# mmdagent/distantspeechrecognition-mirror

Measured on AMD Instinct MI355X. Metric: decoded_audio_hours_per_sec, higher is better.
Workload: dtype f32

## Files before the change

distantspeechrecognition-mirror_amd/csrc/decoder.cpp:

```cpp
#include "common.h"
#include "wfst_graph.h"
#include "lattice.h"
#include "lexicon.h"
#include "wordtrace.h"
#include "viterbi.h"
#include "decode_plan.h"
#include <algorithm>
#include <cmath>

namespace dsr {

static_assert(kPlanSideBytes == (size_t) kSideLds * sizeof(Side), "decode_plan.h budgets the side records of viterbi.h");

struct DecoderState {
  dsr_decoder_cfg cfg; bool haveGraph = false; int nSlots = 0; int nNodes = 0;
  WfstGraph::Csr csr; WfstGraph::Tables tab;
  DevBuf<int> d_xoff, d_xarc, d_xpathOff, d_eoff, d_path, d_nodeFinal, d_queue; DevBuf<float> d_pathCost;
  DevBuf<XRec> d_xrec; DevBuf<ERec> d_erec; DevBuf<float> d_arcCost, d_nodeCost; DevBuf<uint32_t> d_arcOut, d_arcIn;
  DevBuf<TokA> d_tokA, d_ctok; DevBuf<TokB> d_tokB; DevBuf<Side> d_side; DevBuf<XRecD> d_xrecD; int fastOK = 0; int maxCnt = 0; DevBuf<int> d_tokOff, d_tokCnt, d_owner, d_rank, d_chead; DevBuf<unsigned> d_tags; DevBuf<CandA> d_cA; DevBuf<CandB> d_cB; DevBuf<unsigned> d_first; DevBuf<Bp> d_arena;
  DevBuf<long long> d_prof; DevBuf<dsr_decode_result> d_res; DevBuf<int> d_arcs; DevBuf<unsigned> d_words;
  long arenaCap = 0; int initial = 0; unsigned tokenMemoryLimit = 0;
  long lastPoolCap = 0;
  DevBuf<SegState> d_segState; DevBuf<int> d_segDone; DevBuf<unsigned long long> d_poolNext; DevBuf<TokA> d_saveA; DevBuf<TokB> d_saveB;
  DevBuf<WTok> w_tok; DevBuf<WCand> w_cand; DevBuf<int> w_tokOff, w_rank; DevBuf<unsigned long long> w_best; DevBuf<unsigned> w_first; DevBuf<int4> w_traces; size_t w_tablesFor = 0;
  bool costNegZero = false; double costMinAbs = HUGE_VAL;
  DevBuf<uint4> d_lat; DevBuf<double> d_latTtl; DevBuf<long> d_latFrameOff; DevBuf<int> d_arenaLat; DevBuf<int4> d_latFinal; DevBuf<int> d_latInfo;
  int latU = 0, latTmax = 0; long latArenaCap = 0; WfstGraph graphCopy; DevBuf<TokA> d_tokA3; DevBuf<TokB> d_tokB3;
  const dsr_lexicon* lexIn = nullptr; const dsr_lexicon* lexOut = nullptr; uint32_t eosX = 0; std::string eosSymbol;
  int lastU = 0; size_t lastMaxPath = 0; bool lastPaths = false;
  PinBuf<dsr_decode_result> h_res; PinBuf<int> h_arcs; PinBuf<unsigned> h_words; hipEvent_t evDone = nullptr;
  int pendingU = 0; size_t pendingPath = 0; int pendingSlots = 0; long long* pendingProf = nullptr;
  int dumpOn = 0; long dumpCap = 0; DevBuf<long> d_dumpFrameOff, d_dumpCount; DevBuf<int> d_dumpNode, d_dumpArc; DevBuf<float> d_dumpAc, d_dumpLm;
  std::vector<int64_t> h_dumpFrameOff; std::vector<int32_t> h_dumpNode, h_dumpArc; std::vector<float> h_dumpAc, h_dumpLm; int64_t h_dumpFrames = 0;
};

}

using namespace dsr;
struct dsr_decoder : DecoderState {};

extern "C" {

void dsr_decoder_default_cfg(dsr_decoder_cfg* c)
{ memset(c, 0, sizeof(*c)); c->beam = 100.0; c->lmScale = 12.0; c->lmPenalty = 0.0; c->silPenalty = 0.0; c->silenceX = 0xFFFFFFFFu;
  c->propagateN = 5; c->wordTraceLattice = 1; }

dsr_status dsr_decoder_create(const dsr_decoder_cfg* cfg, dsr_decoder** out)
{
  return guard([&] {
    if (!cfg || !out) throw Error(DSR_E_PARAMETER, "null argument");
    require_device();
    dsr_decoder* d = new dsr_decoder(); d->cfg = *cfg;
    if (d->cfg.maxActive <= 0) d->cfg.maxActive = 65536;
    if (d->cfg.maxCandidates <= 0) d->cfg.maxCandidates = 8 * d->cfg.maxActive;
    if (d->cfg.maxCandidates >= (1 << 24)) throw Error(DSR_E_PARAMETER, "maxCandidates must be < 2^24");
    if (d->cfg.streams <= 0) {
      hipDeviceProp_t prop; int dev = 0; DSR_HIP(hipGetDevice(&dev)); DSR_HIP(hipGetDeviceProperties(&prop, dev));
      d->cfg.streams = prop.multiProcessorCount;
      const int t = read_vit_env().slots; if (t > 0) d->cfg.streams = t;
    }
    *out = d;
  });
}
void dsr_decoder_destroy(dsr_decoder* d) { if (d && d->evDone) (void) hipEventDestroy(d->evDone); delete d; }

dsr_status dsr_decoder_set(dsr_decoder* d, const dsr_wfst* g)
{
  return guard([&] {
    if (!d || !g) throw Error(DSR_E_PARAMETER, "null argument");
    if (g->initial < 0) throw Error(DSR_E_CONSISTENCY, "the transducer has no arcs");
    d->csr = g->csr(); d->tab = g->tables(d->csr, (size_t) 1 << 28);
    d->nNodes = (int) g->nodes.size(); d->initial = g->initial; d->graphCopy = *g;
    std::vector<int> nf(d->nNodes); std::vector<float> nc(d->nNodes);
    for (int i = 0; i < d->nNodes; i++) { nf[i] = g->nodes[i].final_; nc[i] = g->nodes[i].cost; }
    d->d_xoff.upload(d->tab.xoff); d->d_eoff.upload(d->tab.eoff); d->d_path.upload(d->tab.path);
    if (d->tab.xrec.empty()) throw Error(DSR_E_CONSISTENCY, "the transducer has no emitting arcs");
    d->d_xrec.upload(d->tab.xrec); d->d_xarc.upload(d->tab.xarc); d->d_xpathOff.upload(d->tab.xpathOff);
    {
      const size_t nx = d->tab.xrec.size(); std::vector<XRecD> xd(nx); int maxCnt = 0; std::vector<float> pc(1, 0.0f);
      for (size_t r = 0; r < nx; r++) {
        const XRec& x = d->tab.xrec[r]; XRecD& o = xd[r];
        o.dst = x.dst; o.dist = x.dist; o.cost = x.cost; o.meta = x.meta; o.dstXoff = d->tab.xoff[x.dst]; o.dstCnt = d->tab.xoff[x.dst + 1] - d->tab.xoff[x.dst];
        const int po = d->tab.xpathOff[r], plen = (int) (x.meta & 0xFFFFu); o.p2 = 0; o.eps1 = 0.0f;
        if (x.meta >> 18) throw Error(DSR_E_CONSISTENCY, "expansion record %zu: meta bits above 17 are in use", r);
        if (plen) { const int a0 = d->tab.path[po]; o.eps1 = d->csr.cost[a0]; if (d->csr.out[a0] != 0) o.meta |= 0x20000u; }
        if (plen > 14) o.meta |= 0x80000000u;
        else if (plen > 1) {
// ... 167 lines not shown
    DSR_HIP(hipMemsetAsync(d->w_best.p, 0xFF, sizeof(unsigned long long) * S * d->nNodes, st)); DSR_HIP(hipMemsetAsync(d->w_first.p, 0xFF, sizeof(unsigned) * S * d->nNodes, st));
  }
  if (maxPath < 1) maxPath = 1;
  d->d_arcs.reserve((size_t) U * maxPath); d->d_words.reserve((size_t) U * maxPath);
  DSR_HIP(hipMemsetAsync(d->d_queue.p, 0, 8 * sizeof(int), st));
  WtArgs A; A.nNodes = d->nNodes; A.initial = d->initial; A.xoff = d->d_xoff.p; A.xrec = d->d_xrec.p; A.xarc = d->d_xarc.p; A.xpathOff = d->d_xpathOff.p; A.eoff = d->d_eoff.p;
  A.erec = d->d_erec.p; A.path = d->d_path.p; A.arcCost = d->d_arcCost.p; A.arcOut = d->d_arcOut.p; A.arcIn = d->d_arcIn.p; A.nodeFinal = d->d_nodeFinal.p; A.nodeCost = d->d_nodeCost.p;
  A.beam = c.beam; A.lmScale = c.lmScale; A.lmPenalty = c.lmPenalty; A.silPenalty = c.silPenalty; A.silenceX = c.silenceX; A.insertSilence = c.insertSilence;
  A.maxTok = c.maxActive; A.maxCand = c.maxCandidates; A.maxTraces = maxTraces;
  A.tok = d->w_tok.p; A.cand = d->w_cand.p; A.tokOff = d->w_tokOff.p; A.rank = d->w_rank.p; A.bestKey = d->w_best.p; A.firstSlot = d->w_first.p; A.traces = d->w_traces.p; A.queue = d->d_queue.p;
  A.scores = score; A.nframes = nframes; A.U = U; A.Tmax = Tmax; A.nDist = nDist; A.res = d->d_res.p; A.arcsOut = d->d_arcs.p; A.wordsOut = d->d_words.p; A.maxPath = maxPath;
  wordtrace_launch(A, slots, st);
  enqueue_result_copies(d, U, want_paths ? (size_t) U * maxPath : 0, st);
  d->pendingSlots = slots; d->pendingProf = nullptr; d->latU = 0;
}

static VitArgs fill_vit_args(dsr_decoder* d, const DecodePlan& P, const VitEnv& env, const float* score, const int32_t* nframes, int U, int Tmax, int nDist,
                             int maxPath, bool wantPaths, hipStream_t st)
{
  const int slots = P.slots; const bool latOn = d->cfg.latticeTokens > 0;
  d->d_res.reserve(U);
  if (wantPaths) { d->d_arcs.reserve((size_t) U * (maxPath > 0 ? maxPath : 1)); d->d_words.reserve((size_t) U * (maxPath > 0 ? maxPath : 1)); }
  DSR_HIP(hipMemsetAsync(d->d_queue.p, 0, 8 * sizeof(int), st));
  if (d->dumpOn) {
    d->dumpCap = (long) d->cfg.maxActive * 64 < (long) 1 << 26 ? (long) 1 << 24 : (long) 1 << 26;
    d->d_dumpFrameOff.reserve(Tmax + 2); d->d_dumpCount.reserve(2);
    d->d_dumpNode.reserve(d->dumpCap); d->d_dumpArc.reserve(d->dumpCap); d->d_dumpAc.reserve(d->dumpCap); d->d_dumpLm.reserve(d->dumpCap);
    DSR_HIP(hipMemsetAsync(d->d_dumpCount.p, 0, 2 * sizeof(long), st));
  }
  VitArgs A; GraphDev& G = A.G; DecDev& D = A.D;
  G.nNodes = d->nNodes; G.initial = d->initial; G.xoff = d->d_xoff.p; G.xrec = d->d_xrec.p; G.xrecD = d->d_xrecD.p; G.xarc = d->d_xarc.p;
  G.xpathOff = d->d_xpathOff.p; G.eoff = d->d_eoff.p; G.erec = d->d_erec.p; G.path = d->d_path.p; G.pathCost = d->d_pathCost.p; G.arcCost = d->d_arcCost.p;
  G.arcOut = d->d_arcOut.p; G.arcIn = d->d_arcIn.p; G.nodeFinal = d->d_nodeFinal.p; G.nodeCost = d->d_nodeCost.p;
  D.beam = d->cfg.beam; D.lmScale = d->cfg.lmScale; D.lmPenalty = d->cfg.lmPenalty; D.silPenalty = d->cfg.silPenalty;
  D.noPen = (d->cfg.lmScale > 0.0 && std::isfinite(d->cfg.lmScale) && d->cfg.lmScale * d->cfg.lmPenalty == 0.0 && d->cfg.lmScale * d->cfg.silPenalty == 0.0 &&
             !d->costNegZero && (d->costMinAbs == HUGE_VAL || d->cfg.lmScale * d->costMinAbs >= 0x1p-60) && !env.pen) ? 1 : 0;
  D.silenceX = d->cfg.silenceX; D.maxTok = d->cfg.maxActive; D.maxCand = d->cfg.maxCandidates; D.arenaCap = d->arenaCap;
  D.tokA = d->d_tokA.p; D.tokB = d->d_tokB.p; D.ctok = d->d_ctok.p; D.side = d->d_side.p; D.fastOK = d->fastOK; D.tokOff = d->d_tokOff.p; D.owner = d->d_owner.p; D.rank = d->d_rank.p; D.cA = d->d_cA.p; D.cB = d->d_cB.p;
  D.first = d->d_first.p; D.tags = d->d_tags.p; D.tokCnt = d->d_tokCnt.p; D.chead = d->d_chead.p; D.arena = d->d_arena.p; D.queue = d->d_queue.p;
  D.segDrop = env.segDrop; D.segQueues = P.segQueues; D.segFrames = P.segFrames; D.segCount = P.segCount;
  D.poolCap = 0; D.poolChunk = 0; D.poolNext = nullptr; D.segState = nullptr; D.segDone = nullptr; D.saveA = nullptr; D.saveB = nullptr;
  if (P.segFrames > 0) {
    d->d_segState.reserve(U); d->d_segDone.reserve(U); d->d_poolNext.reserve(1);
    d->d_saveA.reserve((size_t) U * d->cfg.maxActive); d->d_saveB.reserve((size_t) U * d->cfg.maxActive);
    DSR_HIP(hipMemsetAsync(d->d_segDone.p, 0, sizeof(int) * (size_t) U, st)); DSR_HIP(hipMemsetAsync(d->d_poolNext.p, 0, sizeof(unsigned long long), st));
    D.poolCap = (long) ((size_t) std::max(P.poolArenas, slots) * (size_t) d->arenaCap); if (D.poolCap > (long) 0xFFFFFFF0L) D.poolCap = (long) 0xFFFFFFF0L;
    D.poolChunk = std::min<long>(262144, std::max<long>(4096, D.poolCap / (4 * (long) U)));
    D.poolNext = d->d_poolNext.p; D.segState = d->d_segState.p; D.segDone = d->d_segDone.p; D.saveA = d->d_saveA.p; D.saveB = d->d_saveB.p;
  }
  d->lastPoolCap = D.poolCap;
  D.prof = nullptr;
  if (env.prof) { d->d_prof.reserve((size_t) slots * kProfN); D.prof = d->d_prof.p; }
  D.dumpOn = d->dumpOn; D.dumpCap = d->dumpCap; D.dumpFrameOff = d->d_dumpFrameOff.p; D.dumpNode = d->d_dumpNode.p; D.dumpAc = d->d_dumpAc.p;
  D.dumpLm = d->d_dumpLm.p; D.dumpArc = d->d_dumpArc.p; D.dumpCount = d->d_dumpCount.p;
  D.topN = d->cfg.topN > 0 ? d->cfg.topN : 0; D.tokA3 = nullptr; D.tokB3 = nullptr;
  if (D.topN > 0) { d->d_tokA3.reserve((size_t) slots * d->cfg.maxActive); d->d_tokB3.reserve((size_t) slots * d->cfg.maxActive); D.tokA3 = d->d_tokA3.p; D.tokB3 = d->d_tokB3.p; }
  D.latOn = latOn ? 1 : 0; D.latCap = 0; D.lat = nullptr; D.latTtl = nullptr; D.latFrameOff = nullptr; D.arenaLat = nullptr; D.latFinal = nullptr; D.latInfo = nullptr;
  if (latOn) {
    const size_t cap = (size_t) d->cfg.latticeTokens;
    d->d_lat.reserve((size_t) U * cap); d->d_latTtl.reserve((size_t) U * cap); d->d_latFrameOff.reserve((size_t) U * (Tmax + 3));
    d->d_arenaLat.reserve((size_t) U * (size_t) d->arenaCap); d->d_latFinal.reserve((size_t) U * d->cfg.maxActive); d->d_latInfo.reserve((size_t) 4 * U);
    DSR_HIP(hipMemsetAsync(d->d_latInfo.p, 0, sizeof(int) * 4 * (size_t) U, st));
    D.latCap = (long) cap; D.lat = d->d_lat.p; D.latTtl = d->d_latTtl.p; D.latFrameOff = d->d_latFrameOff.p; D.arenaLat = d->d_arenaLat.p; D.latFinal = d->d_latFinal.p; D.latInfo = d->d_latInfo.p;
    d->latU = U; d->latTmax = Tmax; d->latArenaCap = d->arenaCap;
  } else d->latU = 0;
  A.scores = score; A.nframesArr = nframes; A.U = U; A.Tmax = Tmax; A.nDist = nDist; A.res = d->d_res.p;
  A.arcsOut = wantPaths ? d->d_arcs.p : nullptr; A.wordsOut = wantPaths ? d->d_words.p : nullptr; A.maxPath = maxPath;
  A.useLdsRow = P.useLdsRow; A.hashN = P.hashN; A.regionB = (int) (kSideLds * sizeof(Side)); A.cntCap = P.cntCap;
  return A;
}

dsr_status dsr_decoder_decode_launch(dsr_decoder* d, const float* score, const int32_t* nframes, int U, int Tmax, int nDist,
                                     int maxPath, int want_paths, void* stream)
{
  return guard([&] {
    if (!d || !score || !nframes) throw Error(DSR_E_PARAMETER, "null argument");
    if (!d->haveGraph) throw Error(DSR_E_INITIALIZATION, "call set() with a transducer first");
    if (d->pendingU > 0) throw Error(DSR_E_CONSISTENCY, "a decode is already in flight on this decoder: collect it first");
    if (U <= 0) return;
    hipStream_t st = (hipStream_t) stream;
    if (d->cfg.wordTrace) { launch_wordtrace(d, score, nframes, U, Tmax, nDist, maxPath, want_paths, st); return; }
    check_arc_inputs(d, nDist);
    const bool latOn = d->cfg.latticeTokens > 0;
    if (latOn && d->dumpOn) throw Error(DSR_E_PARAMETER, "lattice bookkeeping and the token dump are separate debugging aids: enable one");
    const VitEnv env = read_vit_env();
    PlanIn in; in.streams = d->cfg.streams; in.maxActive = d->cfg.maxActive; in.arenaTokens = d->cfg.arenaTokens; in.latticeTokens = d->cfg.latticeTokens;
    in.topN = d->cfg.topN; in.dumpOn = d->dumpOn != 0; in.nNodes = d->nNodes; in.maxCnt = d->maxCnt; in.U = U; in.Tmax = Tmax; in.nDist = nDist;
    in.staticLds = viterbi_static_lds(plan_base_modes(in, env));
    const DecodePlan P = plan_decode(in, env, [&] { return xcd_round_robin(st); });
    ensure_scratch(d, P.slots, Tmax, latOn ? U : (P.segFrames > 0 ? P.poolArenas : 0));
    if (maxPath < 0) maxPath = 0;
    const VitArgs A = fill_vit_args(d, P, env, score, nframes, U, Tmax, nDist, maxPath, want_paths != 0, st);
    if (env.segVerbose) fprintf(stderr, "[dsr viterbi] %d utterances on %d workgroups: %s, %s state table\n", U, P.slots, P.segFrames > 0 ? (P.segQueues == 8 ? "time-sliced, XCD-bound queues" : "time-sliced, one queue") : "run to completion", P.narrow ? "narrow" : "wide");
    viterbi_launch(P.modes, A, P.slots, P.ldsBytes, st);
    enqueue_result_copies(d, U, want_paths ? (size_t) U * maxPath : 0, st);
    d->pendingSlots = P.slots; d->pendingProf = A.D.prof;
  });
}

static void report_profile(const long long* prof, int slots)
{
  std::vector<long long> hp((size_t) slots * kProfN); DSR_HIP(hipMemcpy(hp.data(), prof, hp.size() * sizeof(long long), hipMemcpyDeviceToHost));
  double acc[32] = {0}; for (int s2 = 0; s2 < slots; s2++) for (int i = 0; i < 32; i++) acc[i] += (double) hp[(size_t) s2 * kProfN + i];
  fprintf(stderr, "[dsr viterbi prof] mean us per slot:");
  for (int i = 0; i < 32; i++) if (i != 15) fprintf(stderr, " p%d=%.0f", i, acc[i] / slots / 100.0);
  fprintf(stderr, "\n");
  double tmin = 1e30, tmax = 0.0, tsum = 0.0;
  for (int s2 = 0; s2 < slots; s2++) { double t = 0.0; for (int i = 0; i < 32; i++) if (i != 15) t += (double) hp[(size_t) s2 * kProfN + i]; t /= 100.0; tsum += t; if (t < tmin) tmin = t; if (t > tmax) tmax = t; }
  {
    double h[12] = {0}; for (int s2 = 0; s2 < slots; s2++) for (int i = 0; i < 12; i++) h[i] += (double) hp[(size_t) s2 * kProfN + 32 + i];
    const double nf = h[0] + h[1] + h[2] + h[3], tk = h[4] + h[5] + h[6] + h[7];
    static const char* const cn[4] = {"<=8192", "<=12288", ">12288", "memory path"};
    for (int c = 0; c < 4; c++) if (h[c] > 0) fprintf(stderr, "[dsr viterbi prof] frames with %s placements: %.1f %% of the frames, %.1f %% of the frame time, %.1f us per frame, %.2f ns per placement\n",
                                                      cn[c], 100.0 * h[c] / nf, 100.0 * h[4 + c] / tk, h[4 + c] / 100.0 / h[c], h[4 + c] * 10.0 / h[8 + c]);
  }
  fprintf(stderr, "[dsr viterbi prof] busy us per slot: mean %.0f min %.0f max %.0f\n", tsum / slots, tmin, tmax);
  if (slots >= 64 && slots % 8 == 0) {
// ... 163 lines not shown
```

distantspeechrecognition-mirror_amd/csrc/k_viterbi.hip:

```cpp
#include "viterbi.h"
#include <algorithm>
#include <cmath>
#include <type_traits>

namespace dsr {

static constexpr uint32_t kNone = 0xFFFFFFFFu;
static constexpr uint32_t kEndBit = 0x80000000u;
static constexpr int kWaves = kThreads / 64;
static constexpr int kFastK = 8;
static constexpr int kB = 2;
static constexpr int kFastE = 8190;
static constexpr int kP1 = 16;
static constexpr int kW = 4;

typedef const __attribute__((address_space(4))) VitArgs* KP;

__device__ __forceinline__ unsigned ld_u32(const unsigned* p) { return __hip_atomic_load(p, __ATOMIC_RELAXED, __HIP_MEMORY_SCOPE_AGENT); }
__device__ __forceinline__ int ld_i32(const int* p) { return __hip_atomic_load(p, __ATOMIC_RELAXED, __HIP_MEMORY_SCOPE_AGENT); }
__device__ __forceinline__ void st_u32(unsigned* p, unsigned v) { __hip_atomic_store(p, v, __ATOMIC_RELAXED, __HIP_MEMORY_SCOPE_AGENT); }
__device__ __forceinline__ void st_i32(int* p, int v) { __hip_atomic_store(p, v, __ATOMIC_RELAXED, __HIP_MEMORY_SCOPE_AGENT); }
__device__ __forceinline__ void st_u64_dev(void* p, unsigned long long v) { __hip_atomic_store(reinterpret_cast<unsigned long long*>(p), v, __ATOMIC_RELAXED, __HIP_MEMORY_SCOPE_AGENT); }
__device__ __forceinline__ unsigned long long ld_u64_dev(const void* p) { return __hip_atomic_load(reinterpret_cast<const unsigned long long*>(p), __ATOMIC_RELAXED, __HIP_MEMORY_SCOPE_AGENT); }

// ... 92 lines not shown
__global__ __launch_bounds__(kThreads) void k_viterbi(const VitArgs argsInKernarg)
{
  (void) argsInKernarg;
  constexpr bool PROF = (MODES & 1) != 0, EXTRA = (MODES & 2) != 0;
  constexpr bool NARROW = (MODES & 4) != 0;
  const KP KA = (KP) __builtin_amdgcn_kernarg_segment_ptr();
  KP ka = KA;
#define RELOAD() do { ka = KA; asm volatile("" : "+s"(ka)); } while (0)
  RELOAD();
  extern __shared__ __attribute__((aligned(16))) unsigned char smem[];
  float* srow = reinterpret_cast<float*>(smem);
  const int useLdsRow = ka->useLdsRow, nDist = ka->nDist, hashN = ka->hashN, regionB = ka->regionB, cntCap = ka->cntCap;
  unsigned* hkey = reinterpret_cast<unsigned*>(srow + (useLdsRow ? ((nDist + 3) & ~3) : 4));
  unsigned* hfirst = hkey + hashN;
  unsigned* const tab = hkey; const int tabN = NARROW ? 2 * hashN : hashN;
  Side* sideL = reinterpret_cast<Side*>(hfirst + hashN);
  unsigned short* cntL = reinterpret_cast<unsigned short*>(reinterpret_cast<unsigned char*>(hfirst + hashN) + regionB);
  __shared__ int s_waveTot[kWaves];
  __shared__ int s_waveTotE[kWaves];
  __shared__ double s_waveMin[kWaves];
  __shared__ float s_waveMag[kWaves];
  __shared__ unsigned long long s_waveKey[kWaves];
  __shared__ int s_sideN;
  __shared__ int s_tb[2];
  __shared__ unsigned s_bm[kFastC / 32];
  __shared__ unsigned s_gbase[kFastC / 64 + 4];
  __shared__ int s_cnt[(kFastK + 32) * kWaves];
  __shared__ int s_err;
  __shared__ long long s_prof[32]; __shared__ long long s_tlast;
  __shared__ long long s_hist[PROF ? 12 : 1]; __shared__ long long s_tfr;
  __shared__ long long s_stat[3];
  __shared__ int s_maxActive; __shared__ unsigned s_tag; __shared__ long long s_latOff;
  if (PROF && threadIdx.x < 32) s_prof[threadIdx.x] = 0;
  if (PROF && threadIdx.x < 12) s_hist[threadIdx.x] = 0;
#define TICK(ix) do { if (PROF && tid == 0) { const long long tn = (long long) wall_clock64(); s_prof[ix] += tn - s_tlast; s_tlast = tn; } } while (0)
  constexpr int nthr = kThreads, nw = kWaves;
  __shared__ int s_u, s_seg, s_help; __shared__ long long s_chunk;

  const int tid = threadIdx.x;
  const int slot = blockIdx.x;
#define TOKA(ix) ((EXTRA && (ix) == 2) ? ka->D.tokA3 + (size_t) slot * ka->D.maxTok : ka->D.tokA + ((size_t) slot * 2 + (size_t) (ix)) * ka->D.maxTok)
#define TOKB(ix) ((EXTRA && (ix) == 2) ? ka->D.tokB3 + (size_t) slot * ka->D.maxTok : ka->D.tokB + ((size_t) slot * 2 + (size_t) (ix)) * ka->D.maxTok)
#define curA TOKA(bufCur)
#define nxtA TOKA(bufNxt)
#define curB TOKB(bufCur)
#define nxtB TOKB(bufNxt)
#define sprA TOKA(bufSpr)
#define sprB TOKB(bufSpr)
#define ctok (ka->D.ctok + (size_t) slot * 8192)
#define side (ka->D.side + (size_t) slot * kFastC)
#define cA (ka->D.cA + (size_t) slot * ka->D.maxCand)
#define cB (ka->D.cB + (size_t) slot * ka->D.maxCand)
  if (tid == 0) s_tag = ka->D.tags[slot];
#define arena (ka->D.arena + (size_t) ((EXTRA && ka->D.latOn) ? u : (ka->D.segFrames > 0 ? 0 : slot)) * ka->D.arenaCap)
#define sc (ka->scores + (size_t) u * ka->Tmax * nDist)
  constexpr int fastCapC = ((kFastK + 32) * nthr < kFastC) ? (kFastK + 32) * nthr : kFastC;
  constexpr int fastCapN = kP1 * 64 * nw;
  const bool fastOK = ka->D.fastOK && hashN >= 8192;
  const int tableC = (tabN >> 1) + (tabN >> 2), regC = NARROW ? tableC : 2 * tableC, eCap = kFastE, sideLds = regionB >> 5;

  const int nq = (EXTRA || ka->D.segFrames <= 0) ? 1 : ka->D.segQueues;
  const int xcd = nq == 8 ? (int) (__builtin_amdgcn_s_getreg((3 << 11) | 20) & 7u) : 0;
  if (tid == 0) s_help = (nq == 8 && ((ka->D.segDrop >> xcd) & 1)) ? 1 : 0;
  for (;;) {
    __syncthreads();
    if (tid == 0) {
      const int segS0 = EXTRA ? 0 : ka->D.segFrames; int help = s_help, uu = -1, sg = 0;
      for (;;) {
        const int qx = (xcd + help) & (nq - 1), Uq = (ka->U - qx + nq - 1) / nq;
        int it = -1;
        if (help == 0) { it = atomicAdd(ka->D.queue + qx, 1); if (it >= (segS0 > 0 ? ka->D.segCount * Uq : Uq)) it = -1; }
        else {
          int c = ld_i32(ka->D.queue + qx);
          while (c < Uq) { const int prev = atomicCAS(ka->D.queue + qx, c, c + 1); if (prev == c) { it = c; break; } c = prev; }
        }
        if (it >= 0) { uu = segS0 > 0 ? qx + nq * (it % Uq) : it; sg = segS0 > 0 ? it / Uq : 0; break; }
        if (segS0 > 0 && nq == 8 && help < 7) help++; else break;
      }
      if (uu >= 0 && help > 0) { st_i32(&ka->D.segState[uu].status, -2); asm volatile("s_waitcnt vmcnt(0)" ::: "memory"); st_i32(&ka->D.segDone[uu], 0x7FFFFFFF); sg = -1; }
      s_help = help; s_u = uu; s_seg = sg;
    }
    __syncthreads();
    RELOAD();
    const int segS = EXTRA ? 0 : ka->D.segFrames;
    const int u = s_u; if (u < 0) break;
    const bool whole = s_seg < 0; const int seg = whole ? 0 : s_seg;
    const int T = ka->nframesArr[u] < ka->Tmax ? ka->nframesArr[u] : ka->Tmax;
    const int fr0 = seg * segS, frEnd = (segS > 0 && !whole) ? fr0 + segS : 0x7FFFFFFF;
    if (fr0 > T) continue;
    if (EXTRA && ka->D.latOn && tid == 0) ka->D.latFrameOff[(size_t) u * (ka->Tmax + 3)] = 0;
    if (PROF && tid == 0) { const long long tn = (long long) wall_clock64(); if (s_prof[15]) s_prof[10] += tn - s_prof[15]; s_tlast = tn; }
#define dump (EXTRA && ka->D.dumpOn && slot == 0)

    int status = DSR_OK;
// ... 10 lines not shown
        TokB b0; b0.node = ka->G.initial; b0.cnt = ka->G.xoff[ka->G.initial + 1] - ka->G.xoff[ka->G.initial]; curB[0] = b0;
      }
    } else {
      if (tid == 0) { while (ld_i32(&ka->D.segDone[u]) < seg) __builtin_amdgcn_s_sleep(16); }
      __syncthreads();
      if (nq == 1) __builtin_amdgcn_fence(__ATOMIC_ACQUIRE, "agent");
      const SegState* const sst = ka->D.segState + u;
      status = ld_i32(&sst->status);
      if (status != DSR_OK) continue;
      n = ld_i32(&sst->n); arenaOff = (long) ld_u64_dev(&sst->arenaOff); chunkEnd = (long) ld_u64_dev(&sst->chunkEnd); arenaUsed = (long) ld_u64_dev(&sst->arenaUsed); thresh = __longlong_as_double((long long) ld_u64_dev(&sst->thresh));
      if (tid == 0) { s_stat[0] = (long long) ld_u64_dev(&sst->stat[0]); s_stat[1] = (long long) ld_u64_dev(&sst->stat[1]); s_stat[2] = (long long) ld_u64_dev(&sst->stat[2]); s_maxActive = ld_i32(&sst->maxActive); s_latOff = 0; }
      const TokA* const svA = ka->D.saveA + (size_t) u * ka->D.maxTok; const TokB* const svB = ka->D.saveB + (size_t) u * ka->D.maxTok;
      for (int i = tid; i < n; i += nthr) {
        const unsigned long long a0 = ld_u64_dev(&svA[i]), a1 = ld_u64_dev(reinterpret_cast<const unsigned long long*>(&svA[i]) + 1), b0 = ld_u64_dev(&svB[i]);
        unsigned long long* da = reinterpret_cast<unsigned long long*>(&curA[i]); da[0] = a0; da[1] = a1; *reinterpret_cast<unsigned long long*>(&curB[i]) = b0;
      }
    }
    __syncthreads();

    bool cntOK = false;
    int preC = -1;
    const bool preRow = useLdsRow && nDist <= 2 * nthr;
    float rowNext[2] = {0.0f, 0.0f};
    if (preRow && fr0 < T) { const float* r0 = sc + (size_t) fr0 * nDist; if (tid < nDist) rowNext[0] = r0[tid]; if (tid + nthr < nDist) rowNext[1] = r0[tid + nthr]; }
    TICK(11);
    int fr = fr0;
    for (; fr <= T && fr < frEnd && status == DSR_OK; fr++) {
      RELOAD();
      int tidO = (int) threadIdx.x; asm volatile("" : "+v"(tidO));
      const int tid = tidO, lane = tid & 63, wave = tid >> 6;
      const int mode = (fr == T) ? 1 : 0;
      if (mode == 0 && useLdsRow) {
        if (preRow) {
          if (tid < nDist) srow[tid] = rowNext[0];
          if (tid + nthr < nDist) srow[tid + nthr] = rowNext[1];
          if (fr + 1 < T) {
            const float* nr = sc + (size_t) (fr + 1) * nDist;
            if (tid < nDist) rowNext[0] = nr[tid];
            if (tid + nthr < nDist) rowNext[1] = nr[tid + nthr];
          }
        } else { for (int i = tid; i < nDist; i += nthr) srow[i] = sc[(size_t) fr * nDist + i]; }
      }
      const float* rowG = sc + (size_t) fr * nDist;
      int numNew = 0, numStat = -1;
      if (fr > 0) TICK(23);
      if (PROF && tid == 0) { s_tlast = (long long) wall_clock64(); s_tfr = s_tlast; }
      bool fast = fastOK && mode == 0 && n <= fastCapN && !(EXTRA && (ka->D.latOn || ka->D.topN > 0));
// ... 836 lines not shown
          if (tid == 0) { ka->D.dumpFrameOff[fr] = o; ka->D.dumpFrameOff[fr + 1] = o + numNew; cnt[0] = o + numNew; cnt[1] = fr + 1; }
        }
        if (numStat < 0) numStat = numNew;
        if (numStat == 0 || numNew == 0) { status = DSR_E_CONSISTENCY; break; }
        { const int t = bufCur; bufCur = bufNxt; bufNxt = t; }
        n = numNew; arenaOff += numNew; arenaUsed += numNew;
        if (tid == nthr - 1) { s_stat[0] += numStat; s_stat[1] += Cfr; if (fast) s_stat[2] += 1; if (numStat > s_maxActive) s_maxActive = numStat; }
        thresh = __dadd_rn(topScore, ka->D.beam);
      } else {
        const TokA* lst = numNew > 0 ? nxtA : curA; const int cntL = numNew > 0 ? numNew : n;
        unsigned long long key = ~0ull;
        for (int i = tid; i < cntL; i += nthr) {
          const TokA t = lst[i]; const float s = __fadd_rn(t.ac, t.lm);
          if (s == s) { const unsigned long long k = ((unsigned long long) f2ord(s) << 32) | (unsigned) i; if (k < key) key = k; }
        }
        key = wave_min_u64(key);
        if (lane == 0) s_waveKey[wave] = key;
        if (EXTRA && ka->D.latOn) {
          const TokB* lstB = numNew > 0 ? nxtB : curB; int4* lf = ka->D.latFinal + (size_t) u * ka->D.maxTok;
          for (int i = tid; i < cntL; i += nthr) { const TokA t = ld_tok(&lst[i]); lf[i] = make_int4(lstB[i].node, (int) t.bp, __float_as_int(t.ac), __float_as_int(t.lm)); }
          if (tid == 0) { int* li = ka->D.latInfo + 4 * (size_t) u; li[0] = cntL; li[1] = numNew > 0 ? 1 : 0; li[2] = (int) (arenaOff + (numNew > 0 ? numNew : 0)); li[3] = T; }
        }
        __syncthreads();
        int* hopRec = reinterpret_cast<int*>(cB); const int hopCap = 2 * ka->D.maxCand; int* hopOff = hopRec + hopCap;
        if (tid == 0) {
          dsr_decode_result* const res = ka->res;
          clear_result(&res[u]); dsr_decode_result& r = res[u];
          unsigned long long k = ~0ull; for (int w = 0; w < nw; w++) if (s_waveKey[w] < k) k = s_waveKey[w];
          r.frames = T - 1; r.reachedFinal = numNew > 0 ? 1 : 0; r.finalStatesN = numNew;  r.activeHypos = (long) s_stat[0]; r.placements = (long) s_stat[1] + Cfr; r.registerFrames = (long) s_stat[2]; r.maxActiveSeen = s_maxActive; r.status = DSR_OK;
          int nH = 0;
          if (k != ~0ull) {
            const TokA bt = ld_tok(&lst[(unsigned) (k & 0xFFFFFFFFu)]);
            r.ac = bt.ac; r.lm = bt.lm; r.score = __dadd_rn((double) bt.ac, (double) bt.lm);
            for (uint32_t bq = bt.bp; bq != kNone && nH < hopCap; ) {
              uint2 e; if (segS > 0) { const unsigned long long v = ld_u64_dev(&arena[bq]); e.x = (unsigned) v; e.y = (unsigned) (v >> 32); } else e = *reinterpret_cast<const uint2*>(&arena[bq]);
              hopRec[nH++] = (int) e.y; bq = e.x;
            }
          } else r.status = DSR_E_CONSISTENCY;
          s_tb[0] = nH; s_tb[1] = 0;
        }
        __syncthreads();
        const int nH = s_tb[0];
        auto block_excl = [&](const int v, int& total) -> int {
          const int incl = wave_incl_scan(v, lane);
          if (lane == 63) s_waveTot[wave] = incl;
          __syncthreads();
          int base = 0, tot = 0;
          for (int w = 0; w < nw; w++) { const int q = s_waveTot[w]; if (w < wave) base += q; tot += q; }
          __syncthreads();
          total = tot; return base + incl - v;
        };
        int nA = 0;
        for (int b0 = 0; b0 < nH; b0 += nthr) {
          const int i = b0 + tid; int len = 0;
          if (i < nH) { const uint32_t rc = (uint32_t) hopRec[i]; len = (rc & kEndBit) ? ka->G.erec[rc & ~kEndBit].pathLen : (int) (ka->G.xrec[rc].meta & 0xFFFFu) + 1; }
          int total; const int ex = block_excl(len, total);
          if (i < nH) hopOff[i] = nA + ex;
          nA += total;
        }
        int* const arcsOut = ka->arcsOut; unsigned* const wordsOut = ka->wordsOut; const int maxPath = ka->maxPath; dsr_decode_result* const res = ka->res;
        int* ao = arcsOut ? arcsOut + (size_t) u * maxPath : nullptr;
        int nWloc = 0;
        for (int i = tid; i < nH; i += nthr) {
          const uint32_t rc = (uint32_t) hopRec[i]; int pos = nA - hopOff[i];
          if (rc & kEndBit) {
            const ERec e = ka->G.erec[rc & ~kEndBit];
            for (int h = e.pathLen - 1; h >= 0; h--) { const int a = ka->G.path[e.pathOff + h]; pos--; if (ao && pos < maxPath) ao[pos] = a; if (ka->G.arcOut[a] != 0) nWloc++; }
          } else {
            const int a = ka->G.xarc[rc]; pos--; if (ao && pos < maxPath) ao[pos] = a; if (ka->G.arcOut[a] != 0) nWloc++;
            const int pl = (int) (ka->G.xrec[rc].meta & 0xFFFFu); const int po = ka->G.xpathOff[rc];
            for (int h = pl - 1; h >= 0; h--) { const int a2 = ka->G.path[po + h]; pos--; if (ao && pos < maxPath) ao[pos] = a2; if (ka->G.arcOut[a2] != 0) nWloc++; }
          }
        }
        if (nWloc) atomicAdd(&s_tb[1], nWloc);
        __syncthreads();
        if (wordsOut && ao) {
          unsigned* wo = wordsOut + (size_t) u * maxPath; int q = 0;
          const int lim = nA < maxPath ? nA : maxPath;
          for (int b0 = 0; b0 < lim; b0 += nthr) {
            const int i = b0 + tid; unsigned o = 0u;
            if (i < lim) o = ka->G.arcOut[ao[i]];
            int total; const int ex = block_excl(o != 0u ? 1 : 0, total);
            if (o != 0u && q + ex < maxPath) wo[q + ex] = o;
            q += total;
          }
        }
        if (tid == 0) {
          if (res[u].status == DSR_OK) {
            res[u].nArcs = nA; res[u].nWords = s_tb[1];
            if (nH >= hopCap) res[u].status = DSR_E_ALLOCATION; else if (nA > maxPath && arcsOut) res[u].status = DSR_E_DIMENSION;
          }
        }
        __syncthreads();
        TICK(9);
      }
    }

    RELOAD();
    if (PROF && tid == 0) s_prof[15] = (long long) wall_clock64();
    if (segS > 0 && status == DSR_OK && fr <= T) {
      TokA* const svA = ka->D.saveA + (size_t) u * ka->D.maxTok; TokB* const svB = ka->D.saveB + (size_t) u * ka->D.maxTok;
      for (int i = tid; i < n; i += nthr) { svA[i] = curA[i]; svB[i] = curB[i]; }
      if (tid == 0) {
        SegState* const sst = ka->D.segState + u;
        st_i32(&sst->n, n); st_i32(&sst->status, DSR_OK); st_i32(&sst->maxActive, s_maxActive); st_u64_dev(&sst->arenaOff, (unsigned long long) arenaOff); st_u64_dev(&sst->chunkEnd, (unsigned long long) chunkEnd); st_u64_dev(&sst->arenaUsed, (unsigned long long) arenaUsed);
        st_u64_dev(&sst->thresh, (unsigned long long) __double_as_longlong(thresh));
        st_u64_dev(&sst->stat[0], (unsigned long long) s_stat[0]); st_u64_dev(&sst->stat[1], (unsigned long long) s_stat[1]); st_u64_dev(&sst->stat[2], (unsigned long long) s_stat[2]);
      }
      if (nq == 1) __builtin_amdgcn_fence(__ATOMIC_RELEASE, "agent");
      else __builtin_amdgcn_fence(__ATOMIC_RELEASE, "workgroup");
      __syncthreads();
      if (tid == 0) st_i32(&ka->D.segDone[u], seg + 1);
      continue;
    }
    if (status != DSR_OK) {
      if (tid == 0) {
        dsr_decode_result* const res = ka->res; clear_result(&res[u]); res[u].status = status; res[u].frames = T - 1;
        if (segS > 0) { st_i32(&ka->D.segState[u].status, status); asm volatile("s_waitcnt vmcnt(0)" ::: "memory"); st_i32(&ka->D.segDone[u], 0x7FFFFFFF); }
      }
    }
  }
  RELOAD();
  if (tid == 0) ka->D.tags[slot] = s_tag;
  if (PROF && tid < 32) ka->D.prof[slot * kProfN + tid] = s_prof[tid];
  if (PROF && tid < 12) ka->D.prof[slot * kProfN + 32 + tid] = s_hist[tid];
#undef TICK
#undef RELOAD
#undef TOKA
#undef TOKB
#undef curA
#undef nxtA
#undef curB
#undef nxtB
#undef sprA
#undef sprB
#undef ctok
#undef side
#undef cA
#undef cB
#undef arena
// ... 30 lines not shown
```

distantspeechrecognition-mirror_amd/csrc/viterbi.h:

```cpp
#pragma once
#include "common.h"
#include "wfst_graph.h"

namespace dsr {

struct Tok { int32_t node; float ac; float lm; uint32_t bp; };
struct TokA { float ac; float lm; uint32_t bp; uint32_t xs; };
struct TokB { int32_t node; int32_t cnt; };
struct XRecD { int32_t dist; float cost; uint32_t meta; float eps1; int32_t dst; int32_t p2; int32_t dstXoff; int32_t dstCnt; };
struct Side { double ttl; float ac; float lm; int32_t rec; uint32_t prevBp; int32_t c; uint32_t next; };
struct CandA { double ttl; float ac; float lm; };
struct CandB { int32_t dst; int32_t next; int32_t rec; uint32_t prevBp; };
struct Bp { uint32_t prev; uint32_t rec; };
static_assert(sizeof(TokA) == 16 && sizeof(TokB) == 8 && sizeof(XRecD) == 32 && sizeof(Side) == 32 && sizeof(CandA) == 16 && sizeof(CandB) == 16 && sizeof(Bp) == 8,
              "record layouts shared by the host and k_viterbi");

static constexpr int kThreads = 1024;
static constexpr int kFastC = 24576;
static constexpr int kProfN = 48;
static constexpr int kSideLds = 496;

struct GraphDev {
  int nNodes, initial;
  const int* xoff; const XRec* xrec; const XRecD* xrecD; const int* xarc; const int* xpathOff;
  const int* eoff; const ERec* erec; const int* path; const float* pathCost;
  const float* arcCost; const uint32_t* arcOut; const uint32_t* arcIn;
  const int* nodeFinal; const float* nodeCost;
};

struct SegState { int n, status, maxActive, pad; long arenaOff, chunkEnd, arenaUsed; double thresh; long long stat[3]; };

struct DecDev {
  double beam, lmScale, lmPenalty, silPenalty; uint32_t silenceX; int noPen;
  int segFrames, segCount, segQueues, segDrop; long poolCap, poolChunk;    unsigned long long* poolNext; SegState* segState; int* segDone; TokA* saveA; TokB* saveB;
  int maxTok, maxCand; long arenaCap;
  TokA* tokA; TokB* tokB; TokA* ctok; Side* side; int fastOK; int* tokOff; int* tokCnt; int* owner; int* rank; int* chead; CandA* cA; CandB* cB; unsigned* first; unsigned* tags; Bp* arena;
  int* queue; long long* prof;
  int dumpOn; long dumpCap; long* dumpFrameOff; int* dumpNode; float* dumpAc; float* dumpLm; int* dumpArc; long* dumpCount;
  int latOn; long latCap; uint4* lat; double* latTtl; long* latFrameOff; int* arenaLat; int4* latFinal; int* latInfo;
  int topN; TokA* tokA3; TokB* tokB3;
};

struct VitArgs {
  GraphDev G; DecDev D;
  const float* scores; const int* nframesArr; int U, Tmax, nDist;
  dsr_decode_result* res; int* arcsOut; unsigned* wordsOut; int maxPath, useLdsRow, hashN, regionB, cntCap;
};

size_t viterbi_static_lds(int modes);
void viterbi_launch(int modes, const VitArgs& A, int slots, size_t ldsBytes, hipStream_t st);
void xcc_probe_launch(int* out64, hipStream_t st);

}
```

Baseline: 26.37.

## Move path traceback out of Viterbi kernel into separate per-utterance traceback kernel

The backpointer walk, arc-length scan, arc and word emission that used to run at the end of each utterance inside the 1024-thread Viterbi workgroup now run in a new 64-thread traceback kernel with one block per utterance. The Viterbi kernel only records a trace head, and in some modes the hop list, in global memory. A cross-decoder event makes a full-width launch wait for the previous traceback. When there is one utterance per slot, the kernel takes its utterance index directly instead of using the atomic queue. This frees the large workgroup sooner for the next utterance, at the cost of an extra launch, global hop buffers and extra stream ordering.

```diff
diff --git a/distantspeechrecognition-mirror_amd/csrc/decoder.cpp b/distantspeechrecognition-mirror_amd/csrc/decoder.cpp
--- a/distantspeechrecognition-mirror_amd/csrc/decoder.cpp
+++ b/distantspeechrecognition-mirror_amd/csrc/decoder.cpp
@@ -21,6 +21,8 @@
   DevBuf<long long> d_prof; DevBuf<dsr_decode_result> d_res; DevBuf<int> d_arcs; DevBuf<unsigned> d_words;
   long arenaCap = 0; int initial = 0; unsigned tokenMemoryLimit = 0;
   long lastPoolCap = 0;
+  hipEvent_t evTrace = nullptr;
+  DevBuf<TraceHead> d_heads; DevBuf<int> d_hopRec, d_hopOff;
   DevBuf<SegState> d_segState; DevBuf<int> d_segDone; DevBuf<unsigned long long> d_poolNext; DevBuf<TokA> d_saveA; DevBuf<TokB> d_saveB;
   DevBuf<WTok> w_tok; DevBuf<WCand> w_cand; DevBuf<int> w_tokOff, w_rank; DevBuf<unsigned long long> w_best; DevBuf<unsigned> w_first; DevBuf<int4> w_traces; size_t w_tablesFor = 0;
   bool costNegZero = false; double costMinAbs = HUGE_VAL;
@@ -62,7 +64,41 @@
     *out = d;
   });
 }
-void dsr_decoder_destroy(dsr_decoder* d) { if (d && d->evDone) (void) hipEventDestroy(d->evDone); delete d; }
+namespace {
+std::mutex g_traceMu; std::map<int, std::pair<const dsr_decoder*, hipEvent_t>> g_lastTrace; std::map<int, int> g_cuCount;
+void order_behind_last_traceback(int slots, hipStream_t st)
+{
+  std::lock_guard<std::mutex> lock(g_traceMu);
+  int dev = 0; DSR_HIP(hipGetDevice(&dev));
+  auto cu = g_cuCount.find(dev);
+  if (cu == g_cuCount.end()) { int n = 0; DSR_HIP(hipDeviceGetAttribute(&n, hipDeviceAttributeMultiprocessorCount, dev)); cu = g_cuCount.emplace(dev, n).first; }
+  if (slots < cu->second) return;
+  const auto it = g_lastTrace.find(dev);
+  if (it != g_lastTrace.end()) DSR_HIP(hipStreamWaitEvent(st, it->second.second, 0));
+}
+void publish_traceback(dsr_decoder* d, hipStream_t st)
+{
+  std::lock_guard<std::mutex> lock(g_traceMu);
+  if (!d->evTrace) DSR_HIP(hipEventCreateWithFlags(&d->evTrace, hipEventDisableTiming));
+  DSR_HIP(hipEventRecord(d->evTrace, st));
+  int dev = 0; DSR_HIP(hipGetDevice(&dev));
+  g_lastTrace[dev] = std::make_pair((const dsr_decoder*) d, d->evTrace);
+}
+void forget_traceback(const dsr_decoder* d)
+{
+  std::lock_guard<std::mutex> lock(g_traceMu);
+  for (auto it = g_lastTrace.begin(); it != g_lastTrace.end(); ) { if (it->second.first == d) it = g_lastTrace.erase(it); else ++it; }
+}
+}
+
+void dsr_decoder_destroy(dsr_decoder* d)
+{
+  if (!d) return;
+  forget_traceback(d);
+  if (d->evDone) (void) hipEventDestroy(d->evDone);
+  if (d->evTrace) (void) hipEventDestroy(d->evTrace);
+  delete d;
+}
 
 dsr_status dsr_decoder_set(dsr_decoder* d, const dsr_wfst* g)
 {
@@ -276,6 +312,7 @@
   d->d_res.reserve(U);
   if (wantPaths) { d->d_arcs.reserve((size_t) U * (maxPath > 0 ? maxPath : 1)); d->d_words.reserve((size_t) U * (maxPath > 0 ? maxPath : 1)); }
   DSR_HIP(hipMemsetAsync(d->d_queue.p, 0, 8 * sizeof(int), st));
+  d->d_heads.reserve(U); DSR_HIP(hipMemsetAsync(d->d_heads.p, 0xFF, sizeof(TraceHead) * (size_t) U, st));
   if (d->dumpOn) {
     d->dumpCap = (long) d->cfg.maxActive * 64 < (long) 1 << 26 ? (long) 1 << 24 : (long) 1 << 26;
     d->d_dumpFrameOff.reserve(Tmax + 2); d->d_dumpCount.reserve(2);
@@ -321,6 +358,21 @@
   A.scores = score; A.nframesArr = nframes; A.U = U; A.Tmax = Tmax; A.nDist = nDist; A.res = d->d_res.p;
   A.arcsOut = wantPaths ? d->d_arcs.p : nullptr; A.wordsOut = wantPaths ? d->d_words.p : nullptr; A.maxPath = maxPath;
   A.useLdsRow = P.useLdsRow; A.hashN = P.hashN; A.regionB = (int) (kSideLds * sizeof(Side)); A.cntCap = P.cntCap;
+  A.heads = d->d_heads.p;
+  A.hopStride = std::max(1, std::min(2 * D.maxCand, Tmax + 2));
+  d->d_hopRec.reserve((size_t) U * A.hopStride); d->d_hopOff.reserve((size_t) U * A.hopStride); A.hopRec = d->d_hopRec.p;
+  A.oneEach = (P.segFrames == 0 && slots == U) ? 1 : 0;
+  A.walkHere = (P.segFrames == 0 && !latOn && !A.oneEach) ? 1 : 0;
+  return A;
+}
+
+static TraceArgs fill_trace_args(dsr_decoder* d, const VitArgs& V)
+{
+  TraceArgs A; A.hopCap = 2 * V.D.maxCand; A.hopStride = V.hopStride;
+  A.heads = V.heads; A.arena = V.D.arena; A.arenaN = (unsigned long long) d->d_arena.n;
+  A.xrec = V.G.xrec; A.erec = V.G.erec; A.xarc = V.G.xarc; A.xpathOff = V.G.xpathOff; A.path = V.G.path; A.arcOut = V.G.arcOut;
+  A.hopRec = d->d_hopRec.p; A.hopOff = d->d_hopOff.p;
+  A.res = V.res; A.arcsOut = V.arcsOut; A.wordsOut = V.wordsOut; A.maxPath = V.maxPath; A.U = V.U;
   return A;
 }
 
@@ -346,7 +398,11 @@
     if (maxPath < 0) maxPath = 0;
     const VitArgs A = fill_vit_args(d, P, env, score, nframes, U, Tmax, nDist, maxPath, want_paths != 0, st);
     if (env.segVerbose) fprintf(stderr, "[dsr viterbi] %d utterances on %d workgroups: %s, %s state table\n", U, P.slots, P.segFrames > 0 ? (P.segQueues == 8 ? "time-sliced, XCD-bound queues" : "time-sliced, one queue") : "run to completion", P.narrow ? "narrow" : "wide");
+    const TraceArgs TA = fill_trace_args(d, A);
+    order_behind_last_traceback(P.slots, st);
     viterbi_launch(P.modes, A, P.slots, P.ldsBytes, st);
+    traceback_launch(TA, st);
+    publish_traceback(d, st);
     enqueue_result_copies(d, U, want_paths ? (size_t) U * maxPath : 0, st);
     d->pendingSlots = P.slots; d->pendingProf = A.D.prof;
   });
diff --git a/distantspeechrecognition-mirror_amd/csrc/k_traceback.hip b/distantspeechrecognition-mirror_amd/csrc/k_traceback.hip
--- /dev/null
+++ b/distantspeechrecognition-mirror_amd/csrc/k_traceback.hip
@@ -0,0 +1,91 @@
+#include "viterbi.h"
+
+namespace dsr {
+
+static constexpr uint32_t kNone = 0xFFFFFFFFu;
+static constexpr uint32_t kEndBit = 0x80000000u;
+static constexpr int kTraceThreads = 64;
+
+__device__ __forceinline__ int trace_incl_scan(int v)
+{
+  v += __builtin_amdgcn_update_dpp(0, v, 0x111, 0xF, 0xF, true);
+  v += __builtin_amdgcn_update_dpp(0, v, 0x112, 0xF, 0xF, true);
+  v += __builtin_amdgcn_update_dpp(0, v, 0x114, 0xF, 0xF, true);
+  v += __builtin_amdgcn_update_dpp(0, v, 0x118, 0xF, 0xF, true);
+  v += __builtin_amdgcn_update_dpp(0, v, 0x142, 0xA, 0xF, false);
+  v += __builtin_amdgcn_update_dpp(0, v, 0x143, 0xC, 0xF, false);
+  return v;
+}
+
+__global__ __launch_bounds__(kTraceThreads) void k_traceback(const TraceArgs A)
+{
+  const int u = blockIdx.x, lane = threadIdx.x;
+  if (u >= A.U) return;
+  const TraceHead hd = A.heads[u];
+  if (hd.bp == kNone) return;
+  int* const hopRec = A.hopRec + (size_t) u * A.hopStride; int* const hopOff = A.hopOff + (size_t) u * A.hopStride;
+  const int walkCap = A.hopCap < A.hopStride ? A.hopCap : A.hopStride;
+  int nHw = 0;
+  if (hd.hops != kNone) nHw = (int) hd.hops;
+  else if (lane == 0) {
+    const Bp* const arena = A.arena + hd.arenaOff; const unsigned long long arenaN = A.arenaN > hd.arenaOff ? A.arenaN - hd.arenaOff : 0ull;
+    for (uint32_t bq = hd.bp; bq != kNone && nHw < walkCap && bq < arenaN; ) {
+      const uint2 e = *reinterpret_cast<const uint2*>(&arena[bq]);
+      hopRec[nHw++] = (int) e.y; bq = e.x;
+    }
+  }
+  if (nHw > walkCap) nHw = walkCap;
+  const int nH = __builtin_amdgcn_readfirstlane(nHw);
+  __syncthreads();
+  int nA = 0;
+  for (int b0 = 0; b0 < nH; b0 += kTraceThreads) {
+    const int i = b0 + lane; int len = 0;
+    if (i < nH) { const uint32_t rc = (uint32_t) hopRec[i]; len = (rc & kEndBit) ? A.erec[rc & ~kEndBit].pathLen : (int) (A.xrec[rc].meta & 0xFFFFu) + 1; }
+    const int incl = trace_incl_scan(len);
+    if (i < nH) hopOff[i] = nA + incl - len;
+    nA += __builtin_amdgcn_readlane(incl, 63);
+  }
+  const int maxPath = A.maxPath;
+  int* const ao = A.arcsOut ? A.arcsOut + (size_t) u * maxPath : nullptr;
+  int nWloc = 0;
+  for (int i = lane; i < nH; i += kTraceThreads) {
+    const uint32_t rc = (uint32_t) hopRec[i]; int pos = nA - hopOff[i];
+    if (rc & kEndBit) {
+      const ERec e = A.erec[rc & ~kEndBit];
+      for (int h = e.pathLen - 1; h >= 0; h--) { const int a = A.path[e.pathOff + h]; pos--; if (ao && pos < maxPath) ao[pos] = a; if (A.arcOut[a] != 0) nWloc++; }
+    } else {
+      const int a = A.xarc[rc]; pos--; if (ao && pos < maxPath) ao[pos] = a; if (A.arcOut[a] != 0) nWloc++;
+      const int pl = (int) (A.xrec[rc].meta & 0xFFFFu); const int po = A.xpathOff[rc];
+      for (int h = pl - 1; h >= 0; h--) { const int a2 = A.path[po + h]; pos--; if (ao && pos < maxPath) ao[pos] = a2; if (A.arcOut[a2] != 0) nWloc++; }
+    }
+  }
+  const int nW = __builtin_amdgcn_readlane(trace_incl_scan(nWloc), 63);
+  __syncthreads();
+  if (A.wordsOut && ao) {
+    unsigned* const wo = A.wordsOut + (size_t) u * maxPath; int q = 0;
+    const int lim = nA < maxPath ? nA : maxPath;
+    for (int b0 = 0; b0 < lim; b0 += kTraceThreads) {
+      const int i = b0 + lane; unsigned o = 0u;
+      if (i < lim) o = A.arcOut[ao[i]];
+      const int v = o != 0u ? 1 : 0, incl = trace_incl_scan(v);
+      if (o != 0u && q + incl - v < maxPath) wo[q + incl - v] = o;
+      q += __builtin_amdgcn_readlane(incl, 63);
+    }
+  }
+  if (lane == 0) {
+    dsr_decode_result& r = A.res[u];
+    if (r.status == DSR_OK) {
+      r.nArcs = nA; r.nWords = nW;
+      if (nH >= A.hopCap) r.status = DSR_E_ALLOCATION; else if (nA > maxPath && A.arcsOut) r.status = DSR_E_DIMENSION;
+    }
+  }
+}
+
+void traceback_launch(const TraceArgs& A, hipStream_t st)
+{
+  if (A.U <= 0) return;
+  hipLaunchKernelGGL(k_traceback, dim3(A.U), dim3(kTraceThreads), 0, st, A);
+  DSR_HIP(hipGetLastError());
+}
+
+}
diff --git a/distantspeechrecognition-mirror_amd/csrc/k_viterbi.hip b/distantspeechrecognition-mirror_amd/csrc/k_viterbi.hip
--- a/distantspeechrecognition-mirror_amd/csrc/k_viterbi.hip
+++ b/distantspeechrecognition-mirror_amd/csrc/k_viterbi.hip
@@ -138,7 +138,6 @@
   __shared__ float s_waveMag[kWaves];
   __shared__ unsigned long long s_waveKey[kWaves];
   __shared__ int s_sideN;
-  __shared__ int s_tb[2];
   __shared__ unsigned s_bm[kFastC / 32];
   __shared__ unsigned s_gbase[kFastC / 64 + 4];
   __shared__ int s_cnt[(kFastK + 32) * kWaves];
@@ -177,7 +176,7 @@
 
   const int nq = (EXTRA || ka->D.segFrames <= 0) ? 1 : ka->D.segQueues;
   const int xcd = nq == 8 ? (int) (__builtin_amdgcn_s_getreg((3 << 11) | 20) & 7u) : 0;
-  if (tid == 0) s_help = (nq == 8 && ((ka->D.segDrop >> xcd) & 1)) ? 1 : 0;
+  if (tid == 0) { s_help = (nq == 8 && ((ka->D.segDrop >> xcd) & 1)) ? 1 : 0; s_u = -2; }
   for (;;) {
     __syncthreads();
     if (tid == 0) {
@@ -185,7 +184,7 @@
       for (;;) {
         const int qx = (xcd + help) & (nq - 1), Uq = (ka->U - qx + nq - 1) / nq;
         int it = -1;
-        if (help == 0) { it = atomicAdd(ka->D.queue + qx, 1); if (it >= (segS0 > 0 ? ka->D.segCount * Uq : Uq)) it = -1; }
+        if (help == 0) { it = ka->oneEach ? (s_u == -2 ? slot : Uq) : atomicAdd(ka->D.queue + qx, 1); if (it >= (segS0 > 0 ? ka->D.segCount * Uq : Uq)) it = -1; }
         else {
           int c = ld_i32(ka->D.queue + qx);
           while (c < Uq) { const int prev = atomicCAS(ka->D.queue + qx, c, c + 1); if (prev == c) { it = c; break; } c = prev; }
@@ -242,7 +241,10 @@
     int preC = -1;
     const bool preRow = useLdsRow && nDist <= 2 * nthr;
     float rowNext[2] = {0.0f, 0.0f};
-    if (preRow && fr0 < T) { const float* r0 = sc + (size_t) fr0 * nDist; if (tid < nDist) rowNext[0] = r0[tid]; if (tid + nthr < nDist) rowNext[1] = r0[tid + nthr]; }
+    if (preRow && fr0 < T) {
+      const float* r0 = sc + (size_t) fr0 * nDist; int tidU = (int) threadIdx.x; asm volatile("" : "+v"(tidU));
+      if (tidU < nDist) rowNext[0] = r0[tidU]; if (tidU + nthr < nDist) rowNext[1] = r0[tidU + nthr];
+    }
     TICK(11);
     int fr = fr0;
     for (; fr <= T && fr < frEnd && status == DSR_OK; fr++) {
@@ -1125,74 +1127,23 @@
           if (tid == 0) { int* li = ka->D.latInfo + 4 * (size_t) u; li[0] = cntL; li[1] = numNew > 0 ? 1 : 0; li[2] = (int) (arenaOff + (numNew > 0 ? numNew : 0)); li[3] = T; }
         }
         __syncthreads();
-        int* hopRec = reinterpret_cast<int*>(cB); const int hopCap = 2 * ka->D.maxCand; int* hopOff = hopRec + hopCap;
         if (tid == 0) {
           dsr_decode_result* const res = ka->res;
           clear_result(&res[u]); dsr_decode_result& r = res[u];
           unsigned long long k = ~0ull; for (int w = 0; w < nw; w++) if (s_waveKey[w] < k) k = s_waveKey[w];
           r.frames = T - 1; r.reachedFinal = numNew > 0 ? 1 : 0; r.finalStatesN = numNew;  r.activeHypos = (long) s_stat[0]; r.placements = (long) s_stat[1] + Cfr; r.registerFrames = (long) s_stat[2]; r.maxActiveSeen = s_maxActive; r.status = DSR_OK;
-          int nH = 0;
+          TraceHead hd; hd.arenaOff = (unsigned long long) ((size_t) ((EXTRA && ka->D.latOn) ? u : (ka->D.segFrames > 0 ? 0 : slot)) * ka->D.arenaCap);  hd.bp = kNone; hd.hops = kNone;
           if (k != ~0ull) {
             const TokA bt = ld_tok(&lst[(unsigned) (k & 0xFFFFFFFFu)]);
             r.ac = bt.ac; r.lm = bt.lm; r.score = __dadd_rn((double) bt.ac, (double) bt.lm);
-            for (uint32_t bq = bt.bp; bq != kNone && nH < hopCap; ) {
-              uint2 e; if (segS > 0) { const unsigned long long v = ld_u64_dev(&arena[bq]); e.x = (unsigned) v; e.y = (unsigned) (v >> 32); } else e = *reinterpret_cast<const uint2*>(&arena[bq]);
-              hopRec[nH++] = (int) e.y; bq = e.x;
+            hd.bp = bt.bp;
+            if (ka->walkHere) {
+              int* const hopRec = ka->hopRec + (size_t) u * ka->hopStride; const int walkCap = 2 * ka->D.maxCand < ka->hopStride ? 2 * ka->D.maxCand : ka->hopStride; int nH = 0;
+              for (uint32_t bq = bt.bp; bq != kNone && nH < walkCap; ) { const uint2 e = *reinterpret_cast<const uint2*>(&arena[bq]); hopRec[nH++] = (int) e.y; bq = e.x; }
+              hd.hops = (uint32_t) nH;
             }
           } else r.status = DSR_E_CONSISTENCY;
-          s_tb[0] = nH; s_tb[1] = 0;
-        }
-        __syncthreads();
-        const int nH = s_tb[0];
-        auto block_excl = [&](const int v, int& total) -> int {
-          const int incl = wave_incl_scan(v, lane);
-          if (lane == 63) s_waveTot[wave] = incl;
-          __syncthreads();
-          int base = 0, tot = 0;
-          for (int w = 0; w < nw; w++) { const int q = s_waveTot[w]; if (w < wave) base += q; tot += q; }
-          __syncthreads();
-          total = tot; return base + incl - v;
-        };
-        int nA = 0;
-        for (int b0 = 0; b0 < nH; b0 += nthr) {
-          const int i = b0 + tid; int len = 0;
-          if (i < nH) { const uint32_t rc = (uint32_t) hopRec[i]; len = (rc & kEndBit) ? ka->G.erec[rc & ~kEndBit].pathLen : (int) (ka->G.xrec[rc].meta & 0xFFFFu) + 1; }
-          int total; const int ex = block_excl(len, total);
-          if (i < nH) hopOff[i] = nA + ex;
-          nA += total;
-        }
-        int* const arcsOut = ka->arcsOut; unsigned* const wordsOut = ka->wordsOut; const int maxPath = ka->maxPath; dsr_decode_result* const res = ka->res;
-        int* ao = arcsOut ? arcsOut + (size_t) u * maxPath : nullptr;
-        int nWloc = 0;
-        for (int i = tid; i < nH; i += nthr) {
-          const uint32_t rc = (uint32_t) hopRec[i]; int pos = nA - hopOff[i];
-          if (rc & kEndBit) {
-            const ERec e = ka->G.erec[rc & ~kEndBit];
-            for (int h = e.pathLen - 1; h >= 0; h--) { const int a = ka->G.path[e.pathOff + h]; pos--; if (ao && pos < maxPath) ao[pos] = a; if (ka->G.arcOut[a] != 0) nWloc++; }
-          } else {
-            const int a = ka->G.xarc[rc]; pos--; if (ao && pos < maxPath) ao[pos] = a; if (ka->G.arcOut[a] != 0) nWloc++;
-            const int pl = (int) (ka->G.xrec[rc].meta & 0xFFFFu); const int po = ka->G.xpathOff[rc];
-            for (int h = pl - 1; h >= 0; h--) { const int a2 = ka->G.path[po + h]; pos--; if (ao && pos < maxPath) ao[pos] = a2; if (ka->G.arcOut[a2] != 0) nWloc++; }
-          }
-        }
-        if (nWloc) atomicAdd(&s_tb[1], nWloc);
-        __syncthreads();
-        if (wordsOut && ao) {
-          unsigned* wo = wordsOut + (size_t) u * maxPath; int q = 0;
-          const int lim = nA < maxPath ? nA : maxPath;
-          for (int b0 = 0; b0 < lim; b0 += nthr) {
-            const int i = b0 + tid; unsigned o = 0u;
-            if (i < lim) o = ka->G.arcOut[ao[i]];
-            int total; const int ex = block_excl(o != 0u ? 1 : 0, total);
-            if (o != 0u && q + ex < maxPath) wo[q + ex] = o;
-            q += total;
-          }
-        }
-        if (tid == 0) {
-          if (res[u].status == DSR_OK) {
-            res[u].nArcs = nA; res[u].nWords = s_tb[1];
-            if (nH >= hopCap) res[u].status = DSR_E_ALLOCATION; else if (nA > maxPath && arcsOut) res[u].status = DSR_E_DIMENSION;
-          }
+          ka->heads[u] = hd;
         }
         __syncthreads();
         TICK(9);
@@ -1219,6 +1170,7 @@
     if (status != DSR_OK) {
       if (tid == 0) {
         dsr_decode_result* const res = ka->res; clear_result(&res[u]); res[u].status = status; res[u].frames = T - 1;
+        { TraceHead hd; hd.arenaOff = 0ull; hd.bp = kNone; hd.hops = kNone; ka->heads[u] = hd; }
         if (segS > 0) { st_i32(&ka->D.segState[u].status, status); asm volatile("s_waitcnt vmcnt(0)" ::: "memory"); st_i32(&ka->D.segDone[u], 0x7FFFFFFF); }
       }
     }
diff --git a/distantspeechrecognition-mirror_amd/csrc/viterbi.h b/distantspeechrecognition-mirror_amd/csrc/viterbi.h
--- a/distantspeechrecognition-mirror_amd/csrc/viterbi.h
+++ b/distantspeechrecognition-mirror_amd/csrc/viterbi.h
@@ -12,7 +12,8 @@
 struct CandA { double ttl; float ac; float lm; };
 struct CandB { int32_t dst; int32_t next; int32_t rec; uint32_t prevBp; };
 struct Bp { uint32_t prev; uint32_t rec; };
-static_assert(sizeof(TokA) == 16 && sizeof(TokB) == 8 && sizeof(XRecD) == 32 && sizeof(Side) == 32 && sizeof(CandA) == 16 && sizeof(CandB) == 16 && sizeof(Bp) == 8,
+struct TraceHead { unsigned long long arenaOff; uint32_t bp; uint32_t hops; };
+static_assert(sizeof(TokA) == 16 && sizeof(TokB) == 8 && sizeof(XRecD) == 32 && sizeof(Side) == 32 && sizeof(CandA) == 16 && sizeof(CandB) == 16 && sizeof(Bp) == 8 && sizeof(TraceHead) == 16,
               "record layouts shared by the host and k_viterbi");
 
 static constexpr int kThreads = 1024;
@@ -45,10 +46,21 @@
   GraphDev G; DecDev D;
   const float* scores; const int* nframesArr; int U, Tmax, nDist;
   dsr_decode_result* res; int* arcsOut; unsigned* wordsOut; int maxPath, useLdsRow, hashN, regionB, cntCap;
+  TraceHead* heads;
+  int* hopRec; int hopStride, walkHere;
+  int oneEach;
+};
+
+struct TraceArgs {
+  const TraceHead* heads; const Bp* arena; unsigned long long arenaN;
+  const XRec* xrec; const ERec* erec; const int* xarc; const int* xpathOff; const int* path; const uint32_t* arcOut;
+  int* hopRec; int* hopOff; int hopStride, hopCap;
+  dsr_decode_result* res; int* arcsOut; unsigned* wordsOut; int maxPath, U;
 };
 
 size_t viterbi_static_lds(int modes);
 void viterbi_launch(int modes, const VitArgs& A, int slots, size_t ldsBytes, hipStream_t st);
+void traceback_launch(const TraceArgs& A, hipStream_t st);
 void xcc_probe_launch(int* out64, hipStream_t st);
 
 }
```

Result: faster. 26.75, median of 6 (+1.4%).
